# sweeneychris/TheiaSfM

Measured on AMD Instinct MI355X. Metric: ba_observations_per_sec, higher is better.
Workload: dtype f64

## Files before the change

### theiasfm_amd/csrc/device_view.h

```cpp
#pragma once
#include <cstdint>
#include <hip/hip_runtime.h>

namespace tmi {

constexpr int kSpmvTrips = 8;
constexpr unsigned kPinholeDefaultMask = 0x3Fu | (1u << 6) | (1u << 11) | (1u << 12);
constexpr int kWideK = 12;
constexpr int kWideKLarge = 20;
constexpr int kUltraK = 96;

struct DeviceView {
  int Nc, G, Np_pad, nslices, Nrb, D, DP;
  int n_ultra;
  int n_wide;
  int n_track_blocks;
  int Ncam_rb;
  int has_shared;
  int No_pad;
  int Nslots;
  int nub, nnzb;
  int n_order;
  long long npairs;

// ... 43 lines not shown
  const long long* pair_ptr;
  const int* pair_i;
  const int* pair_j;
  const int* ub_order;

  double* pm_r;
  double* pm_A;
  int drop_pos;
  double* pos_coef;
  double* xs;
  int compact;
  int sums_ready;
  double* cp_trk;
  double* xz;
  double* pm_Jp;
  double* pm_A1;
  int planes_fp32;
  double* cam_part;
  double* cm_Y;
  double* cm_A;
  double* cm_R;
  int direct_diag;
  double* trk_rec;
  double* scale_c;
  double* scale_cam;
  double* scale_p;
  double* prep;
  double* prep_c;
  double* Vinv;
  double* gp;
  double* Linv;
  double* Vraw;
  double* yp;
  double* red;
  double* Sdiag;
  double* tbuf;
  double* rbuf;
  double* Minv;
  double* rhs;
  double* yc;
  double* cg_r;
  double* cg_z;
  double* cg_p;
  double* cg_q;
  double* cg_t;
  double* partial;
  double* scal;
  int* flags;
  double* dotbuf;
  int* ticket;
  int* pcg_done;
};

struct HostMirror {
  double scal[32];
  double red[8];
  int flags[8];
  unsigned long long seq;
};

struct RedLayout {
  long long ub, diag, udiag, gt, gc, scalars, total;
};
inline RedLayout red_layout(long long nub, int Nrb, int D) {
  RedLayout L;
  L.ub = 0;
  L.diag = L.ub + nub * D * D;
  L.udiag = L.diag + (long long)Nrb * D * D;
  L.gt = L.udiag + (long long)Nrb * D;
  L.gc = L.gt + (long long)Nrb * D;
  L.scalars = L.gc + (long long)Nrb * D;
  L.total = L.scalars + 8;
  return L;
}

enum {
  SC_COST = 0,
  SC_SS = 1,
  SC_CAND_COST = 2,
  SC_CAND_SS = 3,
  SC_MCC = 4,
  SC_STEP_SQ = 5,
  SC_XNORM_SQ = 6,
  SC_GMAX = 7,
  SC_RHO = 8,
  SC_LAST_RHO = 9,
  SC_PQ = 10,
  SC_ALPHA = 11,
  SC_Q0 = 12,
  SC_Q1 = 13,
  SC_ZETA = 14,
  SC_BNORM = 15,
  SC_GMAX_P = 16,
  SC_RHO_BAD = 17,
  SC_II_DEXT = 18,
  SC_II_DINTR = 19,
  SC_II_XC = 22,
  SC_PCG_STOP = 24,
  SC_COUNT = 32
};
enum { FL_INVALID = 0, FL_SINGULAR_POINT = 1, FL_SINGULAR_BLOCK = 2, FL_PCG_FAIL = 3, FL_CHOL_ABORT = 4, FL_COUNT = 8 };

}
```

### theiasfm_amd/csrc/engine.hip

```cpp
#include <hip/hip_runtime.h>
#include <hip/hip_ext.h>
#include <dlfcn.h>

#include <algorithm>
#include <chrono>
#include <cmath>
#include <cstdio>
#include <cstring>
#include <functional>
#include <mutex>
#include <string>
#include <vector>

#include "../../include/theia_mi355_ba.h"
#include "dense_cholesky.h"
#include "dense_cholesky_df.h"
#include "cluster_chains.h"
#include "cluster_precond.h"
#include "kernels.h"
#include "mf_chunks.h"
#include "direct_diag.h"
#include "pcg_persist.h"
#include "track_kernels.h"
#include "relative_position_kernels.h"
// ... 388 lines not shown
  if (t < FL_COUNT) flags[t] = 0;
  if (t < 8) sc8[t] = 0.0;
}
__global__ void publish_kernel(const double* __restrict__ scal, const double* __restrict__ red8,
                               const int* __restrict__ flags, HostMirror* m, unsigned long long seq) {
  const int t = threadIdx.x;
  if (t < SC_COUNT) m->scal[t] = scal[t];
  if (t < 8) m->red[t] = red8[t];
  if (t < FL_COUNT) m->flags[t] = flags[t];
  __threadfence_system();
  __syncthreads();
  if (t == 0) __hip_atomic_store(&m->seq, seq, __ATOMIC_RELEASE, __HIP_MEMORY_SCOPE_SYSTEM);
}
__global__ void flag_to_scalar_kernel(const int* __restrict__ flag, double* __restrict__ dst) {
  if (threadIdx.x == 0) *dst = (*flag) ? 1.0 : 0.0;
}
}

struct tmi_ba_solver {
  Structure st;
  Launch launch;
  DeviceView v;
  RedLayout RL;
  int DP = 4;
  int device = 0;
  hipStream_t stream = nullptr;
  std::vector<void*> allocs;
  HostMirror* h_mirror = nullptr;
  HostMirror* d_mirror = nullptr;
  unsigned long long mirror_seq = 0;
  double* h_scal = nullptr;
  double* h_red = nullptr;
  int* h_flags = nullptr;
  std::vector<double> ext0, intr0, pts0;
  std::vector<int> grp_off_h;
  double *d_ext0 = nullptr, *d_intr0 = nullptr, *d_pts0 = nullptr;
  int n_intr = 0;
  double* d_pm_u = nullptr;
  double* d_cm_t = nullptr;
  bool need_slot_track = false;
  mfc::View mf = {};
  bool mf_ok = false;
  ddg::Plan dd = {};
  bool direct_ok = false;
  bool fuse_finish_ok = true;
  bool attach_events = true;
  bool pcg_speculate = true;
  bool fast_start_ok = true;
  bool compact_env = true;
  bool fuse_sums = true;
  bool compact_robust = true;
  bool cost_by_view = false;
  bool cost_warm = true;
  bool implicit = false;
  bool adaptive = false;
  bool implicit_now = false;
  bool y_records = false;
  int n_implicit_iterations = 0;
  int adaptive_break_even_override = -1;
  int adaptive_break_even = 4;
  double cur_inv_radius = 0.0;
  double time_vote = 0.0;
  const tmi_ba_options* cur_opts = nullptr;
  double* d_partial_max = nullptr;
  double* d_dense = nullptr;
  double* d_df_tiles = nullptr;
  double* d_df_linv = nullptr;
  int* d_df_flags = nullptr;
  int df_epoch = 0;
  int num_cus = 0;
  clp::Plan cl_plan;
  int shared_diag_chunks = 0;
  double* d_shared_diag_partial = nullptr;
  bool cluster_blocks = false;
  bool cl_built = false;
  int vis_type = 0;
  bool vis_clusters = false;
  std::vector<std::vector<int> > vis_members;
  std::vector<int> vis_cluster_of_rb;
  bool tri = false;
  chains::Segments tri_seg;
  bool cl_failed = false;
  bool cl_active = false;
  bool ppcg_ready = false, ppcg_off = false;
  int ppcg_grid = 0;
  double *d_ppcg_p = nullptr, *d_ppcg_x = nullptr, *d_ppcg_partial = nullptr;
  int* d_ppcg_bar = nullptr;
  long long* d_ppcg_prof = nullptr;
  bool cl_unavailable = false;
  bool cl_retired = false;
  clp::ClusterDesc* d_cl_desc = nullptr;
  clp::GatherEntry* d_cl_ge = nullptr;
  int* d_cl_idx = nullptr;
  double *d_cl_tiles = nullptr, *d_cl_linv = nullptr, *d_cl_vec = nullptr;
  int *d_cl_flags = nullptr, *d_cl_bad = nullptr;
  int cl_epoch = 0;
  int nblocks_slices = 0;
  int nblocks_tracks = 0;
  int nblocks_points = 0;
  tmi_ba_allreduce_fn allreduce = nullptr;
  void* allreduce_user = nullptr;
  void* nccl_comm = nullptr;
  unsigned prof_mask = 0;
  struct Ev { int cls; hipEvent_t a, b; };
  std::vector<Ev> events;
  size_t ev_used = 0;
// ... 50 lines not shown
  int4* d_view_cam = nullptr;
  bool view_index_ready = false;
  int n_order_dev = 0, n_spc_dev = 0;
};

namespace {


template <class T>
int dev_alloc(tmi_ba_solver* s, T** p, size_t n) {
  *p = nullptr;
  if (n == 0) n = 1;
  TMI_HIP(hipMalloc((void**)p, n * sizeof(T)));
  s->allocs.push_back((void*)*p);
  return TMI_BA_OK;
}
template <class T>
int dev_upload(tmi_ba_solver* s, T** p, const std::vector<T>& h) {
  int rc = dev_alloc(s, p, h.size());
  if (rc) return rc;
  if (!h.empty()) TMI_HIP(hipMemcpy(*p, h.data(), h.size() * sizeof(T), hipMemcpyHostToDevice));
  return TMI_BA_OK;
}

struct Timed {
  tmi_ba_solver* s;
  int cls;
  bool on;
  bool attached;
  tmi_ba_solver::Ev* ev = nullptr;
  Timed(tmi_ba_solver* s_, int cls_, bool attach = false) : s(s_), cls(cls_), attached(attach) {
    s->launches[cls]++;
    on = (s->prof_mask >> cls) & 1u;
    if (on) {
      if (s->ev_used == s->events.size()) {
        tmi_ba_solver::Ev e;
        e.cls = cls;
        hipEventCreate(&e.a);
        hipEventCreate(&e.b);
        s->events.push_back(e);
      }
      ev = &s->events[s->ev_used++];
      ev->cls = cls;
      if (!attached) hipEventRecord(ev->a, s->stream);
    }
  }
  hipEvent_t start() const { return on && attached ? ev->a : nullptr; }
  hipEvent_t stop() const { return on && attached ? ev->b : nullptr; }
  ~Timed() {
    if (on && !attached) hipEventRecord(ev->b, s->stream);
  }
};

void select_mirror(tmi_ba_solver* s, int slot) {
  s->h_scal = s->h_mirror[slot].scal;
  s->h_red = s->h_mirror[slot].red;
  s->h_flags = s->h_mirror[slot].flags;
}

int readback(tmi_ba_solver* s) {
  select_mirror(s, 0);
  const unsigned long long seq = ++s->mirror_seq;
  hipLaunchKernelGGL(publish_kernel, dim3(1), dim3(64), 0, s->stream, s->v.scal,
                     s->v.red + s->RL.scalars, s->v.flags, s->d_mirror, seq);
  volatile unsigned long long* p = &s->h_mirror->seq;
  for (unsigned spin = 1;; ++spin) {
    if (*p == seq) break;
    if ((spin & 0xfffu) == 0) {
      const hipError_t q = hipStreamQuery(s->stream);
      if (q == hipSuccess) break;
      if (q != hipErrorNotReady) {
        s->error = std::string("hipStreamQuery: ") + hipGetErrorString(q);
        return TMI_BA_ERR_DEVICE;
      }
    }
    __builtin_ia32_pause();
  }
  __atomic_thread_fence(__ATOMIC_ACQUIRE);
  const hipError_t le = hipGetLastError();
  if (le != hipSuccess) {
    s->error = std::string("kernel launch failed: ") + hipGetErrorString(le);
    return TMI_BA_ERR_DEVICE;
  }
  return TMI_BA_OK;
}

struct Rccl {
  struct Id { char b[128]; };
  int (*GetUniqueId)(void*) = nullptr;
  int (*CommInitRank)(void**, int, Id, int) = nullptr;
  int (*AllReduce)(const void*, void*, size_t, int, int, void*, hipStream_t) = nullptr;
  int (*CommDestroy)(void*) = nullptr;
  const char* (*GetErrorString)(int) = nullptr;
  bool ok = false;
  std::string error;
};
Rccl& rccl() {
  static Rccl r;
  static bool tried = false;
  if (tried) return r;
  tried = true;
  void* h = nullptr;
  const char* names[] = {"librccl.so", "librccl.so.1", "/opt/rocm/lib/librccl.so.1", "/opt/rocm/lib/librccl.so"};
  for (const char* n : names)
    if ((h = dlopen(n, RTLD_NOW | RTLD_NOLOAD))) break;
  if (!h)
// ... 1353 lines not shown
  TMI_HIP(hipMemsetAsync(v.pcg_done, 0, sizeof(int), s->stream));
  TMI_HIP(hipMemsetAsync(v.cg_q, 0, (size_t)(n_r + 8) * sizeof(double), s->stream));
  TMI_HIP(hipMemsetAsync(v.yc, 0, std::max(n_r, 1) * sizeof(double), s->stream));
  TMI_HIP(hipMemsetAsync(v.red, 0, s->RL.total * sizeof(double), s->stream));
  TMI_HIP(hipMemsetAsync(v.cm_Y, 0, (v.write_y ? (size_t)std::max<int64_t>(st.Nslots, 1) * YS : 1) * sizeof(double), s->stream));
  TMI_HIP(hipMemsetAsync(v.cm_A, 0, (size_t)std::max<int64_t>(st.Nslots, 1) * AS * sizeof(double), s->stream));
  {
    int* orb;
    if ((rc = dev_alloc(s, &orb, (size_t)std::max<int64_t>(st.No_pad, 1)))) return rc;
    if (st.No_pad > 0)
      hipLaunchKernelGGL(obs_rb_kernel, dim3((unsigned)((st.No_pad + 255) / 256)), dim3(256), 0, s->stream, v.obs_cam, v.cam_rb,
                         st.Nc, (long long)st.No_pad, orb);
    v.obs_rb = orb;
  }
  if (s->need_slot_track && !st.has_shared) {
    rc = build_mf_chunks(s);
    if (rc) return rc;
  }
  v.drop_pos = 0;
  const bool two_pass_possible = (s->implicit || s->adaptive) && !s->mf_ok;
  if (!light && !two_pass_possible && !st.has_shared && O->residual_precision != 32 && D >= 3 && s->DP >= 3) {
    const char* e = getenv("TMI_BA_DROP_POS");
    bool ok = !(e && atoi(e) == 0);
    for (int rb = 0; rb < st.Nrb && ok; ++rb) {
      const int c = st.rb_cam[rb];
      ok = c >= 0 && (st.cam_mask[c] & 7u) == 7u;
    }
    for (int lp = 0; lp < st.Np_pad && ok; ++lp) ok = st.pt_const[lp] == 0;
    if (ok) {
      if ((rc = dev_alloc(s, &v.pos_coef, (size_t)3 * std::max(st.Np_pad, 1)))) return rc;
      if ((rc = dev_alloc(s, &v.cp_trk, (size_t)7 * std::max(st.Np_pad, 1)))) return rc;
      if ((rc = dev_alloc(s, &v.xs, (size_t)std::max(st.Nrb, 1) * D + 8))) return rc;
      if ((rc = dev_alloc(s, &v.xz, (size_t)std::max(st.Nrb, 1) * D + 8))) return rc;
      v.drop_pos = 1;
    }
  }
  if (setup_timing) fprintf(stderr, "[tmi_ba setup] position columns of the A planes: %s\n", v.drop_pos ? "formed from Jp" : "stored");
  s->direct_ok = false;
  {
    const char* env = getenv("TMI_BA_FUSED_FINISH");
    s->fuse_finish_ok = !(env && env[0] == '0');
    env = getenv("TMI_BA_ATTACH_EVENTS");
    s->attach_events = !(env && env[0] == '0');
    env = getenv("TMI_BA_PCG_SPECULATE");
    s->pcg_speculate = !(env && env[0] == '0');
    env = getenv("TMI_BA_FAST_START");
    s->fast_start_ok = !(env && env[0] == '0');
    env = getenv("TMI_BA_COMPACT_PLANES");
    s->compact_env = !(env && env[0] == '0');
    env = getenv("TMI_BA_FUSE_TRACK_SUMS");
    s->fuse_sums = !(env && env[0] == '0');
    env = getenv("TMI_BA_COMPACT_ROBUST");
    s->compact_robust = !(env && env[0] == '0');
  }
  v.direct_diag = 0;
  {
    const char* e = getenv("TMI_BA_DIRECT_DIAG");
    if (s->mf_ok && !st.has_shared && O->residual_precision != 32 && !s->cluster_blocks && st.Nrb > 0 && st.Nslots > 0 && D <= ddg::kMaxD &&
        !(e && atoi(e) == 0)) {
      std::vector<int> cp((size_t)st.Nrb + 1);
      TMI_HIP(hipMemcpyAsync(cp.data(), v.cam_ptr, cp.size() * sizeof(int), hipMemcpyDeviceToHost, s->stream));
      TMI_HIP(hipStreamSynchronize(s->stream));
      std::vector<int> crb, cs0, cs1, rbc((size_t)st.Nrb + 1, 0);
      for (int rb = 0; rb < st.Nrb; ++rb) {
        rbc[rb] = (int)crb.size();
        const int n = cp[rb + 1] - cp[rb];
        if (n <= 0) continue;
        const int nch = (n + ddg::kChunkSlots - 1) / ddg::kChunkSlots;
        const int per = (((n + nch - 1) / nch) + 63) & ~63;
        for (int b = cp[rb]; b < cp[rb + 1]; b += per) {
          crb.push_back(rb);
          cs0.push_back(b);
          cs1.push_back(std::min(b + per, cp[rb + 1]));
        }
      }
      rbc[st.Nrb] = (int)crb.size();
      int *p0, *p1, *p2, *p3, *stt;
      double *xy, *part;
      if ((rc = dev_upload(s, &p0, crb))) return rc;
      if ((rc = dev_upload(s, &p1, cs0))) return rc;
      if ((rc = dev_upload(s, &p2, cs1))) return rc;
      if ((rc = dev_upload(s, &p3, rbc))) return rc;
      if ((rc = dev_alloc(s, &xy, (size_t)2 * st.Nslots))) return rc;
      if ((rc = dev_alloc(s, &part, std::max<size_t>(crb.size(), 1) * ddg::n_acc(D)))) return rc;
      if ((rc = dev_alloc(s, &v.trk_rec, (size_t)std::max(st.Np_pad, 1) * ddg::trk_stride(s->DP)))) return rc;
      if ((rc = dev_alloc(s, &stt, (size_t)st.Nslots))) return rc;
      hipLaunchKernelGGL(ddg::slot_gather_kernel, dim3(s->nblocks_tracks), dim3(256), 0, s->stream, v, stt, xy);
      v.slot_track = stt;
      s->dd.n_chunks = (int)crb.size();
      s->dd.chunk_rb = p0;
      s->dd.chunk_s0 = p1;
      s->dd.chunk_s1 = p2;
      s->dd.rb_chunk = p3;
      s->dd.cm_xy = xy;
      s->dd.part = part;
      s->direct_ok = true;
      const char* ec = getenv("TMI_BA_COST_BY_VIEW");
      if (const char* ew = getenv("TMI_BA_COST_WARM")) s->cost_warm = atoi(ew) != 0;
      s->cost_by_view = st.Nslots == st.No && ((int)crb.size() + 3) / 4 <= nbmax && !(ec && atoi(ec) == 0);
    }
  }
  if (s->adaptive) {
    const double form = (s->DP == 4 ? 79.0 : 61.0) * (double)st.npairs + (s->direct_ok ? 80.0 * (double)st.No : 0.0),
                 with_s = 195.0 * (double)st.nub,
                 free = (s->mf_ok ? (s->DP == 4 ? 57.0 : 52.0) : 85.0) * (double)st.No;
    if (const char* e = getenv("TMI_BA_BREAK_EVEN")) s->adaptive_break_even_override = atoi(e);
// ... 874 lines not shown
  hipStream_t stream = s->stream;
  s->prof_mask = (O->profile_kernels == 1) ? 0xffffffffu : (unsigned)O->profile_kernels;
  s->cl_retired = false;
  s->ev_used = 0;
  memset(s->launches, 0, sizeof(s->launches));
  sum->num_reduced_blocks = st.Nrb;
  sum->reduced_block_dim = D;
  sum->num_schur_blocks = st.nub + st.Nrb;
  sum->num_schur_pairs = st.npairs;
  sum->setup_time_in_seconds = s->setup_seconds;
  int rc;
#define CK(x) if ((rc = (x)) != TMI_BA_OK) return fail(rc)
#define CKH(call) do { hipError_t e_ = (call); if (e_ != hipSuccess) { s->error = std::string(#call) + ": " + hipGetErrorString(e_); return fail(TMI_BA_ERR_DEVICE); } } while (0)

  const int lt = O->loss_function_type;
  const double lw = O->robust_loss_width;
  const bool iterative = (O->linear_solver_type == TMI_BA_ITERATIVE_SCHUR || O->linear_solver_type == TMI_BA_CGNR);
  s->cur_opts = O;
  if (iterative && (s->st.has_shared || s->vis_clusters) &&
      ((s->tri && O->preconditioner_type == TMI_BA_PRECOND_CLUSTER_JACOBI) ||
       (!s->tri && O->preconditioner_type == TMI_BA_PRECOND_CLUSTER_TRIDIAGONAL && st.world == 1 && !s->implicit))) {
    s->error = "CLUSTER_JACOBI / CLUSTER_TRIDIAGONAL: the solver was created for the other one";
    return fail(TMI_BA_ERR_INVALID_ARGUMENT);
  }
  if (iterative && s->vis_clusters &&
      (O->preconditioner_type == TMI_BA_PRECOND_CLUSTER_JACOBI || O->preconditioner_type == TMI_BA_PRECOND_CLUSTER_TRIDIAGONAL) &&
      O->visibility_clustering_type != s->vis_type) {
    s->error = "visibility_clustering_type differs from the value the solver was created with";
    return fail(TMI_BA_ERR_INVALID_ARGUMENT);
  }
  if (s->implicit && !iterative) {
    s->error = "this solver was created for the implicit Schur operator (ITERATIVE_SCHUR); "
               "an exact linear solver type needs schur_mode = explicit at creation";
    return fail(TMI_BA_ERR_INVALID_ARGUMENT);
  }
  double* d_sc = v.red + RL.scalars;

  CKH(hipMemsetAsync(v.flags, 0, FL_COUNT * sizeof(int), stream));
  CKH(hipMemsetAsync(v.yc, 0, std::max(n_r, 1) * sizeof(double), stream));
  hipLaunchKernelGGL(fill_kernel, dim3((n_r + 255) / 256 + 1), dim3(256), 0, stream, v.scale_c, (long long)n_r, 1.0);
  s->launch.expand_scale(v, stream);
  prepare_cameras(s, v.ext, v.intr, v.prep);
  hipLaunchKernelGGL(fill_kernel, dim3((unsigned)(((long long)st.Np_pad * s->DP + 255) / 256 + 1)), dim3(256), 0, stream, v.scale_p, (long long)st.Np_pad * s->DP, 1.0);
  bool compact_possible = s->compact_env && v.drop_pos && v.uniform_pinhole_default && s->mf_ok && s->direct_ok && D == 9 &&
                          (lt == 0 || s->compact_robust) && iterative && !s->cluster_blocks && v.cp_trk != nullptr && !v.planes_fp32;
  if (compact_possible) {
    compact_possible = (int)s->grp_off_h.size() == st.G + 1;
    for (int g = 0; g < st.G && compact_possible; ++g) {
      const double* K = s->intr0.data() + s->grp_off_h[g];
      compact_possible = s->grp_off_h[g + 1] - s->grp_off_h[g] >= 7 && K[1] == 1.0 && K[2] == 0.0;
    }
  }
  int last_pcg_len = 0;
  auto linearize = [&](bool norms_only = false, bool full_planes = false) {
    if (!norms_only)
      v.compact = (!full_planes && compact_possible && (s->implicit || (s->adaptive && last_pcg_len <= s->adaptive_break_even)))
                      ? (lt == 0 ? 1 : 2)
                      : 0;
    if (!norms_only) v.sums_ready = (v.compact && s->fuse_sums) ? 1 : 0;
    Timed t(s, TMI_BA_K_LINEARIZE);
    s->launch.linearize(v, stream, v.prep, lt, lw, nbs, d_sc, norms_only ? 1 : 0);
  };
  v.direct_diag = (s->direct_ok && iterative) ? 1 : 0;
  const bool fast_start = O->jacobi_scaling && v.direct_diag && s->fast_start_ok;
  linearize(fast_start, O->jacobi_scaling != 0);
  hipLaunchKernelGGL(flag_to_scalar_kernel, dim3(1), dim3(64), 0, stream, v.flags + FL_INVALID, d_sc + 2);
  CK(do_allreduce(s, d_sc, 8));
  CK(readback(s));
  double hsc[8];
  memcpy(hsc, s->h_red, sizeof(hsc));
  const int64_t No_global_hint = st.No;
  (void)No_global_hint;
  if (hsc[2] > 0.0) {
    s->error = "residual evaluation failed at the start point (a track lies on a camera centre)";
    return fail(TMI_BA_ERR_EVALUATION_FAILED);
  }
  double cost = hsc[0];
  double n_obs_global = (double)st.No;
  if (st.world > 1) {
    double tmp[8] = {(double)st.No, 0, 0, 0, 0, 0, 0, 0};
    CKH(hipMemcpyAsync(d_sc, tmp, sizeof(tmp), hipMemcpyHostToDevice, stream));
    CK(do_allreduce(s, d_sc, 8));
    CKH(hipMemcpyAsync(tmp, d_sc, sizeof(tmp), hipMemcpyDeviceToHost, stream));
    CKH(hipStreamSynchronize(stream));
    n_obs_global = tmp[0];
  }
  sum->initial_cost = cost;
  sum->initial_rmse = n_obs_global > 0 ? std::sqrt(hsc[1] / n_obs_global) : 0.0;
  double final_ss = hsc[1];

  auto trial_cost = [&]() {
    if (s->cost_by_view) {
      const int nb = (s->dd.n_chunks + 3) / 4;
      hipLaunchKernelGGL(ddg::cost_view_kernel, dim3(nb), dim3(256), 0, stream, v, s->dd, v.prep_c, v.pts_c, lt, lw, FL_INVALID,
                         nb, v.partial, d_sc + 3, d_sc + 5, s->cost_warm ? 1 : 0);
    } else {
      s->launch.cost(v, stream, v.prep_c, v.pts_c, lt, lw, FL_INVALID, nbs, v.partial, d_sc + 3, d_sc + 5);
    }
  };
  auto build_camera_side = [&](double inv_radius, bool skip_direct_reduce = false) {
    {
      Timed t(s, TMI_BA_K_POINT_ELIMINATE);
      s->launch.point_eliminate(v, stream, inv_radius, O->min_lm_diagonal, O->max_lm_diagonal, nbs,
                                s->d_partial_max, d_sc + 6, O->gradient_tolerance, st.world > 1 ? d_sc + 0 : nullptr);
    }
    {
      Timed t(s, TMI_BA_K_CAMERA_DIAG);
      if (v.direct_diag) {
        s->launch.camera_diag_direct(v, stream, RL, s->dd, v.prep, lt, lw, skip_direct_reduce ? 1 : 0);
      } else {
        s->launch.camera_diag(v, stream, RL, s->shared_diag_chunks, s->d_shared_diag_partial);
        s->launch.shared_blocks(v, stream, RL);
      }
    }
  };
  if (O->jacobi_scaling) {
    if (fast_start) {
      Timed t(s, TMI_BA_K_CAMERA_DIAG);
      s->launch.track_records_points_only(v, stream, v.pts);
      s->launch.camera_diag_direct(v, stream, RL, s->dd, v.prep, lt, lw, 0);
    } else {
      {
        Timed t(s, TMI_BA_K_REDUCE);
        s->launch.point_scale(v, stream, nbs);
      }
      build_camera_side(1.0);
    }
    CK(do_allreduce(s, v.red + RL.udiag, n_r));
    {
      Timed t(s, TMI_BA_K_REDUCE);
      if (n_r) {
        CKH(hipMemcpyAsync(v.scale_c, v.red + RL.udiag, (size_t)n_r * sizeof(double), hipMemcpyDeviceToDevice, stream));
        hipLaunchKernelGGL(camera_scale_finish_kernel, dim3((n_r + 255) / 256), dim3(256), 0, stream, v.scale_c, n_r);
        s->launch.expand_scale(v, stream);
        prepare_cameras(s, v.ext, v.intr, v.prep);
      }
    }
    linearize();
  }
  double xnorm_cam_sq = 0.0, xnorm_pts_sq = 0.0;
  {
    Timed t(s, TMI_BA_K_UPDATE_COST);
    s->launch.update_cameras(v, stream, v.scal + SC_STEP_SQ, v.prep_c);
    hipLaunchKernelGGL(points_norm_kernel, dim3(nbp), dim3(256), 0, stream, v, v.pts, nbp, v.partial, d_sc);
  }
  CK(do_allreduce(s, d_sc, 8));
  CK(readback(s));
  memcpy(hsc, s->h_red, sizeof(hsc));
  xnorm_cam_sq = s->h_scal[SC_STEP_SQ + 1];
  xnorm_pts_sq = hsc[0];
  double x_norm = std::sqrt(xnorm_cam_sq + xnorm_pts_sq);

  const double t_loop = now_s();
  double radius = O->initial_trust_region_radius;
  double decrease_factor = 2.0;
  int invalid_run = 0;
  int iter = 0;
  int termination = 1;
  const char* why = "maximum number of iterations reached";
  int64_t pcg_iters = 0;
  s->n_implicit_iterations = 0;
  bool need_gradient_check = true;
  bool inner_enabled = O->use_inner_iterations != 0;
  bool time_up = false;

  for (;;) {
    if (iter >= O->max_num_iterations) break;
    if (st.world > 1 ? time_up : (now_s() - t_start >= O->max_solver_time_in_seconds)) {
      why = "maximum solver time reached";
      break;
    }
    ++iter;
    const double inv_radius = 1.0 / radius;
    const double radius_used = radius;
    const int64_t pcg_before = pcg_iters;
    auto trace = [&](double outcome, double cand, double mcc, double step) {
      if (!O->iteration_trace || iter > O->iteration_trace_capacity) return;
      double* row = O->iteration_trace + (size_t)(iter - 1) * TMI_BA_TRACE_STRIDE;
      row[0] = iter; row[1] = cost; row[2] = radius_used; row[3] = outcome; row[4] = cand; row[5] = mcc;
      row[6] = (double)(pcg_iters - pcg_before); row[7] = step;
    };
    hipLaunchKernelGGL(iteration_begin_kernel, dim3(1), dim3(64), 0, stream, v.flags, d_sc);
    s->cur_inv_radius = inv_radius;
    if (s->adaptive && iterative && !s->st.has_shared) {
      s->implicit_now = last_pcg_len <= s->adaptive_break_even;
      if (s->y_records) v.write_y = s->implicit_now ? 0 : 1;
      if (s->implicit_now) s->n_implicit_iterations++;
    } else if (s->implicit && iterative) {
      s->n_implicit_iterations++;
    }
    v.direct_diag = (s->direct_ok && iterative && s->implicit_now && !s->cluster_blocks) ? 1 : 0;
    if (v.compact && !v.direct_diag) {
      compact_possible = false;
      linearize();
      hipLaunchKernelGGL(iteration_begin_kernel, dim3(1), dim3(64), 0, stream, v.flags, d_sc);
    }
    const bool cluster_handle = s->st.has_shared || s->vis_clusters;
    const bool cluster_precond = O->preconditioner_type == TMI_BA_PRECOND_CLUSTER_JACOBI ||
                                 O->preconditioner_type == TMI_BA_PRECOND_CLUSTER_TRIDIAGONAL;
    const bool fuse_finish = s->fuse_finish_ok && iterative && n_r > 0 && !(cluster_handle && cluster_precond);
    const bool fuse_direct = fuse_finish && v.direct_diag && st.world == 1;
    build_camera_side(inv_radius, fuse_direct);
    if (!s->implicit_now || s->cluster_blocks) {
      Timed t(s, TMI_BA_K_SCHUR_OFFDIAG);
      s->launch.schur_offdiag(v, stream, RL);
      s->launch.cross_add(v, stream, RL);
    }
    CK(do_allreduce(s, v.red, RL.total));
    const int precond_mode = O->preconditioner_type == TMI_BA_PRECOND_IDENTITY ? 1
                             : O->preconditioner_type == TMI_BA_PRECOND_SCHUR_JACOBI_PARAMETER_BLOCKS ? 2 : 0;
    if (fuse_finish) {
      Timed t(s, TMI_BA_K_PRECONDITIONER);
      s->launch.camera_finish(v, stream, RL, s->dd, inv_radius, O->min_lm_diagonal, O->max_lm_diagonal,
                              need_gradient_check ? 1 : 0, precond_mode, fuse_direct ? 1 : 0);
      s->cl_active = false;
    } else {
      Timed t(s, TMI_BA_K_REDUCE);
// ... 14 lines not shown
            (void)hipGetLastError();
            s->error.clear();
            s->cl_unavailable = true;
            s->cl_active = false;
          } else if (rc != TMI_BA_OK) {
            return fail(rc);
          }
        }
      }
      const int64_t before = pcg_iters;
      if (s->cl_active && s->cl_failed) {
        usable = 0;
      } else {
        CK(solve_reduced_pcg(s, O, &usable, &pcg_iters, fuse_finish));
      }
      last_pcg_len = (int)(pcg_iters - before);
      sum->effective_preconditioner_type =
          s->cl_active ? (s->tri ? TMI_BA_PRECOND_CLUSTER_TRIDIAGONAL : TMI_BA_PRECOND_CLUSTER_JACOBI)
          : O->preconditioner_type == TMI_BA_PRECOND_IDENTITY ? TMI_BA_PRECOND_IDENTITY
          : O->preconditioner_type == TMI_BA_PRECOND_SCHUR_JACOBI_PARAMETER_BLOCKS ? TMI_BA_PRECOND_SCHUR_JACOBI_PARAMETER_BLOCKS
                                                                                    : TMI_BA_PRECOND_SCHUR_JACOBI;
    } else {
      CK(solve_reduced_dense(s, &usable));
    }
    if (!(iterative && n_r > 0)) {
      CK(readback(s));
      if (!iterative && s->h_flags[FL_CHOL_ABORT]) {
        TMI_HIP(hipMemsetAsync(v.flags + FL_CHOL_ABORT, 0, sizeof(int), stream));
        {
          Timed t(s, TMI_BA_K_CHOLESKY);
          CK(solve_reduced_dense_panels(s));
        }
        CK(readback(s));
      }
    }
    if (s->h_red[6] > 0.0 || s->h_flags[FL_SINGULAR_BLOCK]) usable = 0;
    if (need_gradient_check) {
      double vote = (s->h_scal[SC_GMAX] > O->gradient_tolerance) ? 1.0 : 0.0;
      if (st.world > 1)
        vote += s->h_red[0];
      else
        vote += (s->h_scal[SC_GMAX_P] > O->gradient_tolerance) ? 1.0 : 0.0;
      need_gradient_check = false;
      if (vote == 0.0) {
        termination = 0;
        why = "gradient tolerance reached";
        --iter;
        break;
      }
    }
    double model_cost_change = 0.0, step_sq = 0.0, cand_cost = 0.0, cand_ss = 0.0;
    double cand_xc_sq = 0.0, cand_xp_sq = 0.0;
    bool cand_invalid = false;
    if (usable) {
      {
        Timed t(s, TMI_BA_K_UPDATE_COST);
        s->launch.update_cameras(v, stream, v.scal + SC_STEP_SQ, v.prep_c);
      }
      {
        Timed t(s, TMI_BA_K_BACK_SUBSTITUTE);
        s->launch.back_substitute(v, stream, nbs, v.partial, d_sc + 0);
      }
      {
        Timed t(s, TMI_BA_K_UPDATE_COST);
        trial_cost();
      }
      if (st.world > 1 && now_s() - t_start >= O->max_solver_time_in_seconds) {
        s->time_vote = 1.0;
        CKH(hipMemcpyAsync(d_sc + 7, &s->time_vote, sizeof(double), hipMemcpyHostToDevice, stream));
      }
      CK(do_allreduce(s, d_sc, 8));
      CK(readback(s));
      memcpy(hsc, s->h_red, sizeof(hsc));
      time_up = st.world > 1 && hsc[7] > 0.0;
      model_cost_change = hsc[0];
      step_sq = hsc[1] + s->h_scal[SC_STEP_SQ];
      cand_xp_sq = hsc[2];
      cand_xc_sq = s->h_scal[SC_STEP_SQ + 1];
      cand_cost = hsc[3];
      cand_ss = hsc[4];
      cand_invalid = hsc[5] > 0.0;
      if (!(model_cost_change > 0.0)) usable = 0;
    }
    bool inner_useful = false;
    if (usable && inner_enabled && !cand_invalid) {
      CK(run_inner_sweep(s, O));
      {
        Timed t(s, TMI_BA_K_UPDATE_COST);
        CKH(hipMemsetAsync(v.flags + FL_INVALID, 0, sizeof(int), stream));
        prepare_cameras(s, v.ext_c, v.intr_c, v.prep_c);
        trial_cost();
        hipLaunchKernelGGL(diff_sq_kernel, dim3(1), dim3(1024), 0, stream, v.ext, v.ext_c, (long long)6 * st.Nc, v.scal + SC_II_DEXT);
        hipLaunchKernelGGL(diff_sq_kernel, dim3(1), dim3(1024), 0, stream, v.intr, v.intr_c, (long long)s->n_intr, v.scal + SC_II_DINTR);
        hipLaunchKernelGGL(points_diff_kernel, dim3(nbp), dim3(256), 0, stream, v, nbp, v.partial);
        hipLaunchKernelGGL(reduce_sum_kernel, dim3(2), dim3(256), 0, stream, v.partial, nbp, d_sc + 1);
        hipLaunchKernelGGL(cameras_norm_kernel, dim3(1), dim3(1024), 0, stream, v, v.scal + SC_II_XC);
      }
      CK(do_allreduce(s, d_sc, 8));
      CK(readback(s));
      const double inner_cost = s->h_red[3], inner_ss = s->h_red[4];
      if (s->h_red[5] > 0.0) {
        CKH(hipMemcpyAsync(v.ext_c, s->inner.bak_ext, (size_t)6 * st.Nc * sizeof(double), hipMemcpyDeviceToDevice, stream));
        if (s->n_intr) CKH(hipMemcpyAsync(v.intr_c, s->inner.bak_intr, (size_t)s->n_intr * sizeof(double), hipMemcpyDeviceToDevice, stream));
        CKH(hipMemcpyAsync(v.pts_c, s->inner.bak_pts, (size_t)4 * st.Np_pad * sizeof(double), hipMemcpyDeviceToDevice, stream));
        prepare_cameras(s, v.ext_c, v.intr_c, v.prep_c);
      } else {
        model_cost_change += cand_cost - inner_cost;
        inner_useful = inner_cost < cost;
        inner_enabled = (1.0 - inner_cost / cand_cost) > 1e-3;
        cand_cost = inner_cost;
        cand_ss = inner_ss;
        step_sq = s->h_scal[SC_II_DEXT] + s->h_scal[SC_II_DINTR] + s->h_red[1];
        cand_xc_sq = s->h_scal[SC_II_XC];
        cand_xp_sq = s->h_red[2];
        sum->num_inner_iteration_steps++;
      }
    }
    if (!usable) {
      trace(-1.0, std::nan(""), model_cost_change, 0.0);
      sum->num_unsuccessful_steps++;
      if (++invalid_run >= O->max_num_consecutive_invalid_steps) {
        termination = 2;
        why = "too many consecutive invalid steps";
        break;
      }
      radius /= decrease_factor;
      decrease_factor *= 2.0;
      if (radius < O->min_trust_region_radius) {
        termination = 0;
        why = "minimum trust region radius reached";
        break;
      }
      continue;
    }
    invalid_run = 0;
    if (cand_invalid) cand_cost = 1.7976931348623157e308;
    const double step_norm = std::sqrt(step_sq);
    if (step_norm <= O->parameter_tolerance * (x_norm + O->parameter_tolerance)) {
      trace(2.0, cand_cost, model_cost_change, step_norm);
      termination = 0;
      why = "parameter tolerance reached";
      break;
    }
    const double cost_change = cost - cand_cost;
    if (std::fabs(cost_change) <= O->function_tolerance * cost) {
      trace(3.0, cand_cost, model_cost_change, step_norm);
      termination = 0;
      why = "function tolerance reached";
      break;
    }
    const double relative_decrease = cost_change / model_cost_change;
    trace((inner_useful || relative_decrease > O->min_relative_decrease) ? 1.0 : 0.0, cand_cost, model_cost_change, step_norm);
    if (inner_useful || relative_decrease > O->min_relative_decrease) {
      std::swap(v.ext, v.ext_c);
      std::swap(v.intr, v.intr_c);
      std::swap(v.pts, v.pts_c);
      std::swap(v.prep, v.prep_c);
      cost = cand_cost;
      final_ss = cand_ss;
      x_norm = std::sqrt(cand_xc_sq + cand_xp_sq);
      sum->num_successful_steps++;
      radius = radius / std::fmax(1.0 / 3.0, 1.0 - std::pow(2.0 * relative_decrease - 1.0, 3));
      radius = std::fmin(O->max_trust_region_radius, radius);
      decrease_factor = 2.0;
      linearize();
      need_gradient_check = true;
    } else {
      sum->num_unsuccessful_steps++;
      radius /= decrease_factor;
      decrease_factor *= 2.0;
    }
    if (radius < O->min_trust_region_radius) {
      termination = 0;
      why = "minimum trust region radius reached";
      break;
    }
    if (O->verbose && st.rank == 0)
      fprintf(stderr, "[tmi_ba] it %3d cost %.10e radius %.3e pcg %lld\n", iter, cost, radius, (long long)pcg_iters);
  }
  CKH(hipStreamSynchronize(stream));
  const double t_end = now_s();
  (void)t_loop;

  sum->termination = termination;
  sum->num_iterations = iter;
  sum->num_linear_solver_iterations = pcg_iters;
  sum->num_matrix_free_iterations = s->n_implicit_iterations;
  sum->final_cost = cost;
  sum->final_rmse = n_obs_global > 0 ? std::sqrt(final_ss / n_obs_global) : 0.0;
  sum->success = (termination != 2);
  sum->status = (termination == 2) ? TMI_BA_ERR_LINEAR_SOLVER : TMI_BA_OK;
  sum->solve_time_in_seconds = t_end - t_start;
  set_message(sum, why);
  for (int c = 0; c < TMI_BA_NUM_KERNEL_CLASSES; ++c) sum->kernel_launches[c] = s->launches[c];
  for (size_t i = 0; i < s->ev_used; ++i) {
    float ms = 0.f;
    if (s->events[i].cls < 0) continue;
    if (hipEventElapsedTime(&ms, s->events[i].a, s->events[i].b) == hipSuccess)
      sum->kernel_seconds[s->events[i].cls] += 1e-3 * ms;
  }
  return sum->status;
#undef CK
#undef CKH
}

int32_t tmi_ba_solve(tmi_ba_problem* P, const tmi_ba_options* O, tmi_ba_summary* sum) {
  if (!P || !O || !sum) return TMI_BA_ERR_INVALID_ARGUMENT;
  tmi_ba_solver* s = nullptr;
  memset(sum, 0, sizeof(*sum));
  const int rc = tmi_ba_solver_create(P, O, 0, 1, &s);
  if (rc != TMI_BA_OK) {
    sum->status = rc;
    sum->termination = 2;
    set_message(sum, g_last_error.empty() ? tmi_ba_status_string(rc) : g_last_error.c_str());
    return rc;
  }
  const int rc2 = tmi_ba_solver_solve(s, O, sum);
  if (sum->success) tmi_ba_solver_download(s, P);
  tmi_ba_solver_destroy(s);
  return rc2;
// ... 1377 lines not shown
  int64_t psum = 0;
  for (int64_t k = 0; k < st.npairs; ++k)
    psum += (slot_obs[st.pair_i[k]] + 1) * 31 + (slot_obs[st.pair_j[k]] + 1) * 17;
  out[11] = psum;
  return TMI_BA_OK;
}

int32_t tmi_ba_solver_structure_checksums(tmi_ba_solver* s, uint64_t out[24]) {
  if (!s || !out) return TMI_BA_ERR_INVALID_ARGUMENT;
  TMI_HIP(hipSetDevice(s->device));
  TMI_HIP(hipStreamSynchronize(s->stream));
  const Structure& st = s->st;
  const DeviceView& v = s->v;
  auto sum = [&](const void* dev, size_t bytes, uint64_t* dst) -> int {
    std::vector<unsigned char> h(bytes);
    if (bytes) TMI_HIP(hipMemcpy(h.data(), dev, bytes, hipMemcpyDeviceToHost));
    uint64_t x = 1469598103934665603ULL;
    for (unsigned char c : h) x = (x ^ c) * 1099511628211ULL;
    *dst = x;
    return TMI_BA_OK;
  };
  int rc;
  memset(out, 0, 24 * sizeof(uint64_t));
  out[0] = s->device_structure ? 1 : 0;
  const size_t Npad = (size_t)st.Np_pad, Nop = (size_t)st.No_pad, Nrb = (size_t)st.Nrb, nub = (size_t)st.nub;
#define CS(i, ptr, n, T) if ((rc = sum(ptr, (size_t)(n) * sizeof(T), &out[i]))) return rc;
  CS(1, v.slice_ptr, st.nslices + 1, int) CS(2, v.pt_k, Npad, int) CS(3, v.pt_const, Npad, unsigned char)
  CS(4, v.obs_cam, Nop, int) CS(5, v.obs_xy, 2 * Nop, double) CS(6, v.obs_cpos, Nop, int)
  CS(7, v.cam_ptr, Nrb + 1, int) CS(20, s->d_pt_orig, Npad, int)
  if (!s->light && !s->implicit) {
    CS(8, v.ub_i, nub, int) CS(9, v.ub_j, nub, int) CS(10, v.urow_ptr, Nrb + 1, int) CS(11, v.ucol_ptr, Nrb + 1, int)
    CS(12, v.ucol_u, nub, int) CS(13, v.spc_row, v.n_spc, int) CS(14, v.spc_u0, v.n_spc, int)
    CS(15, v.spc_rptr, Nrb + 1, int) CS(16, v.pair_ptr, nub + 1, long long) CS(17, v.pair_i, st.npairs, int)
    CS(18, v.pair_j, st.npairs, int) CS(19, v.ub_order, (size_t)v.n_order * 4, int)
  }
#undef CS
  out[21] = (uint64_t)v.n_order;
  out[22] = (uint64_t)v.n_spc;
  out[23] = (uint64_t)st.Nslots;
  return TMI_BA_OK;
}

int32_t tmi_ba_solver_operator_info(tmi_ba_solver* s, int32_t out[8]) {
  if (!s || !out) return TMI_BA_ERR_INVALID_ARGUMENT;
  for (int i = 0; i < 8; ++i) out[i] = 0;
  out[0] = s->mf_ok ? 1 : 0;
  out[1] = s->v.drop_pos ? 1 : 0;
  out[2] = s->direct_ok ? 1 : 0;
  out[3] = s->adaptive ? 1 : 0;
  out[4] = s->implicit ? 1 : 0;
  out[5] = s->adaptive ? (int32_t)std::min(s->adaptive_break_even, 1 << 30) : 0;
  out[6] = ((s->st.has_shared || s->vis_clusters) && !s->cl_unavailable) ? 1 : 0;
  out[7] = s->v.compact ? 1 : 0;
  return TMI_BA_OK;
}

int32_t tmi_ba_solver_evaluate(tmi_ba_solver* s, double* residuals, double* jac_camera,
                               double* jac_shared, double* jac_point, uint8_t* valid,
                               int32_t* block_dim) {
  if (!s || s->light) return TMI_BA_ERR_INVALID_ARGUMENT;
  TMI_HIP(hipSetDevice(s->device));
  {
    const int rcm = materialize_host_layout(s);
    if (rcm) return rcm;
  }
  DeviceView& v = s->v;
  Structure& st = s->st;
  const int D = st.D, DP = s->DP;
  const int n_r = st.Nrb * D;
  hipStream_t stream = s->stream;
  if (block_dim) *block_dim = D;
  TMI_HIP(hipMemsetAsync(v.flags, 0, FL_COUNT * sizeof(int), stream));
  hipLaunchKernelGGL(fill_kernel, dim3((n_r + 255) / 256 + 1), dim3(256), 0, stream, v.scale_c, (long long)n_r, 1.0);
  s->launch.expand_scale(v, stream);
  prepare_cameras(s, v.ext, v.intr, v.prep);
  hipLaunchKernelGGL(fill_kernel, dim3((unsigned)(((long long)st.Np_pad * DP + 255) / 256 + 1)), dim3(256), 0, stream, v.scale_p, (long long)st.Np_pad * DP, 1.0);
  {
    DeviceView ve = v;
    ve.drop_pos = 0;
    ve.compact = 0;
    v.compact = 0;
    v.sums_ready = 0;
    s->launch.linearize(ve, stream, v.prep, 0, 1.0, s->nblocks_tracks, nullptr, 0);
  }
  const size_t N = (size_t)st.No_pad;
  std::vector<double> r(residuals ? 2 * N : 0), A(jac_camera ? (size_t)2 * D * N : 0),
      Jp(jac_point ? (size_t)2 * DP * N : 0);
  if (residuals) TMI_HIP(hipMemcpyAsync(r.data(), v.pm_r, r.size() * sizeof(double), hipMemcpyDeviceToHost, stream));
  if (jac_camera) TMI_HIP(hipMemcpyAsync(A.data(), v.pm_A, A.size() * sizeof(double), hipMemcpyDeviceToHost, stream));
  if (jac_point) TMI_HIP(hipMemcpyAsync(Jp.data(), v.pm_Jp, Jp.size() * sizeof(double), hipMemcpyDeviceToHost, stream));
  std::vector<double> A1((jac_shared && st.has_shared) ? (size_t)2 * D * N : 0);
  if (!A1.empty()) TMI_HIP(hipMemcpyAsync(A1.data(), v.pm_A1, A1.size() * sizeof(double), hipMemcpyDeviceToHost, stream));
  TMI_HIP(hipStreamSynchronize(stream));
  if (v.planes_fp32) {
    auto widen = [](std::vector<double>& buf) {
      std::vector<float> f(buf.size());
      if (!f.empty()) memcpy(f.data(), buf.data(), f.size() * sizeof(float));
      for (size_t k = 0; k < f.size(); ++k) buf[k] = (double)f[k];
    };
    widen(r); widen(A); widen(Jp); widen(A1);
  }
  for (size_t e = 0; e < N; ++e) {
    const int64_t i = st.obs_orig[e];
    if (i < 0) continue;
    auto at = [e](int npl, int plane) {
      return (e >> 6) * (size_t)(npl * 64) + (size_t)(plane >> 1) * 128 + ((e & 63) << 1) + (size_t)(plane & 1);
    };
    if (residuals) {
      residuals[2 * i] = r[at(2, 0)];
      residuals[2 * i + 1] = r[at(2, 1)];
    }
    if (jac_camera)
      for (int a = 0; a < D; ++a) {
        jac_camera[(size_t)2 * D * i + a] = A[at(2 * D, 2 * a)];
        jac_camera[(size_t)2 * D * i + D + a] = A[at(2 * D, 2 * a + 1)];
      }
    if (jac_shared)
      for (int a = 0; a < D; ++a) {
        jac_shared[(size_t)2 * D * i + a] = A1.empty() ? 0.0 : A1[at(2 * D, 2 * a)];
        jac_shared[(size_t)2 * D * i + D + a] = A1.empty() ? 0.0 : A1[at(2 * D, 2 * a + 1)];
      }
    if (jac_point)
      for (int a = 0; a < DP; ++a) {
        jac_point[(size_t)2 * DP * i + a] = Jp[at(2 * DP, 2 * a)];
        jac_point[(size_t)2 * DP * i + DP + a] = Jp[at(2 * DP, 2 * a + 1)];
      }
    if (valid) valid[i] = 1;
  }
  if (valid) {
// ... 24 lines not shown
```

### theiasfm_amd/lib.py

```python
from __future__ import annotations

import ctypes as C
import os

import numpy as np

from . import abi

_HERE = os.path.dirname(os.path.abspath(__file__))
LIB_PATH = os.path.join(_HERE, "lib", "libtheia_mi355_ba.so")
_lib = None

EXPORTS = (
    "tmi_ba_version", "tmi_ba_device_count", "tmi_ba_status_string", "tmi_ba_last_error",
    "tmi_ba_options_init",
    "tmi_ba_intrinsics_size", "tmi_ba_intrinsics_constant_mask", "tmi_ba_solve",
    "tmi_ba_solver_create", "tmi_ba_solver_set_allreduce", "tmi_ba_solver_solve",
    "tmi_ba_solver_reset", "tmi_ba_solver_set_parameters", "tmi_ba_solver_download", "tmi_ba_solver_stream",
    "tmi_ba_solver_destroy", "tmi_ba_solver_evaluate", "tmi_ba_structure_stats", "tmi_ba_structure_stats_for",
    "tmi_ba_rccl_unique_id", "tmi_ba_solver_init_rccl", "tmi_ba_solver_debug_allreduce",
    "tmi_ba_solver_filter_outlier_tracks", "tmi_ba_filter_outlier_tracks",
    "tmi_ba_solver_adjust_tracks", "tmi_ba_adjust_tracks",
    "tmi_ba_solver_adjust_views", "tmi_ba_adjust_views",
    "tmi_ba_track_estimator_options_init", "tmi_ba_solver_estimate_tracks", "tmi_ba_estimate_tracks",
# ... 425 lines not shown
            min_num_optimized_tracks_per_view, None if vm is None else vm.ctypes.data, sel.ctypes.data, ln.ctypes.data, err.ctypes.data,
            C.byref(ss))
        if st != 0:
            raise EngineError(st, "tmi_ba_solver_select_good_tracks")
        return sel, ln, err, ss

    def adjust_tracks(self, options: abi.COptions):
        n = self.problem.num_points
        term = np.full(n, -1, dtype=np.int8)
        iters = np.zeros(n, dtype=np.int32)
        c0 = np.zeros(n)
        c1 = np.zeros(n)
        ts = abi.CTrackBatchSummary()
        st = self._L.tmi_ba_solver_adjust_tracks(self._h, C.byref(options), term.ctypes.data,
                                                 iters.ctypes.data, c0.ctypes.data, c1.ctypes.data,
                                                 C.byref(ts))
        if st != 0:
            raise EngineError(st, "tmi_ba_solver_adjust_tracks")
        return term, iters, c0, c1, ts

    def adjust_views(self, options: abi.COptions, view_mask=None):
        vm, term, iters, c0, c1, vs = _view_outputs(self.problem.num_cameras, view_mask)
        st = self._L.tmi_ba_solver_adjust_views(self._h, C.byref(options), None if vm is None else vm.ctypes.data,
                                                term.ctypes.data, iters.ctypes.data, c0.ctypes.data, c1.ctypes.data,
                                                C.byref(vs))
        if st != 0:
            raise EngineError(st, "tmi_ba_solver_adjust_views")
        return term, iters, c0, c1, vs

    def estimate_tracks(self, estimator_options: abi.CTrackEstimatorOptions, ba_options: abi.COptions,
                        track_mask=None):
        tm, status, es = _track_mask(self.problem.num_points, track_mask)
        st = self._L.tmi_ba_solver_estimate_tracks(self._h, C.byref(estimator_options), C.byref(ba_options),
                                                   None if tm is None else tm.ctypes.data, status.ctypes.data,
                                                   C.byref(es))
        if st != 0:
            raise EngineError(st, "tmi_ba_solver_estimate_tracks")
        return status, es

    def structure_checksums(self):
        out = (C.c_uint64 * 24)()
        st = self._L.tmi_ba_solver_structure_checksums(self._h, out)
        if st != 0:
            raise EngineError(st, "tmi_ba_solver_structure_checksums")
        return list(out)

    def operator_info(self) -> dict:
        out = (C.c_int32 * 8)()
        st = self._L.tmi_ba_solver_operator_info(self._h, out)
        if st != 0:
            raise EngineError(st, "tmi_ba_solver_operator_info")
        return dict(one_sweep_product=bool(out[0]), position_columns_formed=bool(out[1]), direct_camera_side=bool(out[2]),
                    adaptive=bool(out[3]), implicit=bool(out[4]), break_even=int(out[5]), cluster_handle=bool(out[6]),
                    compact_planes=bool(out[7]))

    @property
    def stream(self) -> int:
        return int(self._L.tmi_ba_solver_stream(self._h) or 0)

    def evaluate(self, point_dof: int):
        n = self.problem.num_observations
        bd = C.c_int32(0)
        r = np.zeros((n, 2))
        A = np.zeros(n * 2 * 16)
        A1 = np.zeros(n * 2 * 16)
        Jp = np.zeros((n, 2, point_dof))
        valid = np.zeros(n, dtype=np.uint8)
        st = self._L.tmi_ba_solver_evaluate(self._h, r.ctypes.data, A.ctypes.data, A1.ctypes.data,
                                            Jp.ctypes.data, valid.ctypes.data, C.byref(bd))
        if st != 0:
            raise EngineError(st, "tmi_ba_solver_evaluate")
        D = bd.value
        return r, A[: n * 2 * D].reshape(n, 2, D), A1[: n * 2 * D].reshape(n, 2, D), Jp, valid, D

    def close(self):
        if self._h:
            self._L.tmi_ba_solver_destroy(self._h)
            self._h = C.c_void_p()

    def __del__(self):
        try:
            self.close()
        except Exception:
            pass
```

Before: 2.474 billion.

## Speculatively linearize at the candidate point into a second buffer set

When the step evaluation would use compact planes, the candidate cost is computed by a full linearization at the candidate parameters into a second set of residual/Jacobian/track buffers, instead of a separate trial-cost pass. If the step is accepted, the buffer sets are swapped, so the linearization after acceptance is not recomputed. The cost is extra device memory and wasted linearization work on rejected steps. It is gated on direct-diag mode, no inner iterations and the previous step having succeeded.

```diff
diff --git a/theiasfm_amd/csrc/device_view.h b/theiasfm_amd/csrc/device_view.h
--- a/theiasfm_amd/csrc/device_view.h
+++ b/theiasfm_amd/csrc/device_view.h
@@ -119,6 +119,24 @@
   int* pcg_done;
 };
 
+struct LinearisationSet {
+  double* pm_r;
+  double* pm_A;
+  double* pm_Jp;
+  double* cp_trk;
+  double* Vraw;
+  double* gp;
+};
+inline void swap_linearisation_set(DeviceView& v, LinearisationSet& o) {
+  double* t;
+  t = v.pm_r, v.pm_r = o.pm_r, o.pm_r = t;
+  t = v.pm_A, v.pm_A = o.pm_A, o.pm_A = t;
+  t = v.pm_Jp, v.pm_Jp = o.pm_Jp, o.pm_Jp = t;
+  t = v.cp_trk, v.cp_trk = o.cp_trk, o.cp_trk = t;
+  t = v.Vraw, v.Vraw = o.Vraw, o.Vraw = t;
+  t = v.gp, v.gp = o.gp, o.gp = t;
+}
+
 struct HostMirror {
   double scal[32];
   double red[8];
diff --git a/theiasfm_amd/csrc/engine.hip b/theiasfm_amd/csrc/engine.hip
--- a/theiasfm_amd/csrc/engine.hip
+++ b/theiasfm_amd/csrc/engine.hip
@@ -464,6 +464,10 @@
   bool compact_robust = true;
   bool cost_by_view = false;
   bool cost_warm = true;
+  bool spec_env = true;
+  bool spec_ready = false, spec_off = false;
+  bool spec_swapped = false;
+  LinearisationSet spec_set = {nullptr, nullptr, nullptr, nullptr, nullptr, nullptr};
   bool implicit = false;
   bool adaptive = false;
   bool implicit_now = false;
@@ -620,6 +624,32 @@
   }
 };
 
+void primary_linearisation_set(tmi_ba_solver* s) {
+  if (!s->spec_swapped) return;
+  swap_linearisation_set(s->v, s->spec_set);
+  s->spec_swapped = false;
+}
+bool ensure_speculative_set(tmi_ba_solver* s) {
+  if (s->spec_ready) return true;
+  if (s->spec_off) return false;
+  const size_t N = std::max<size_t>((size_t)s->st.No_pad, 1), NP = std::max<size_t>((size_t)s->st.Np_pad, 1);
+  const size_t DP = (size_t)s->DP, NS = (size_t)sym_size(s->DP);
+  const size_t n[6] = {2 * N, 4 * N, 2 * DP * N, 7 * NP, NS * NP, DP * NP};
+  double* p[6] = {nullptr, nullptr, nullptr, nullptr, nullptr, nullptr};
+  for (int i = 0; i < 6; ++i) {
+    if (hipMalloc((void**)&p[i], n[i] * sizeof(double)) != hipSuccess) {
+      (void)hipGetLastError();
+      for (int j = 0; j < i; ++j) (void)hipFree(p[j]);
+      s->spec_off = true;
+      return false;
+    }
+  }
+  for (int i = 0; i < 6; ++i) s->allocs.push_back((void*)p[i]);
+  s->spec_set = LinearisationSet{p[0], p[1], p[2], p[3], p[4], p[5]};
+  s->spec_ready = true;
+  return true;
+}
+
 void select_mirror(tmi_ba_solver* s, int slot) {
   s->h_scal = s->h_mirror[slot].scal;
   s->h_red = s->h_mirror[slot].red;
@@ -2079,6 +2109,8 @@
     s->fuse_sums = !(env && env[0] == '0');
     env = getenv("TMI_BA_COMPACT_ROBUST");
     s->compact_robust = !(env && env[0] == '0');
+    env = getenv("TMI_BA_SPECULATIVE_LINEARIZE");
+    s->spec_env = !(env && env[0] == '0');
   }
   v.direct_diag = 0;
   {
@@ -3059,11 +3091,17 @@
     }
   }
   int last_pcg_len = 0;
+  auto compact_now = [&](bool full_planes) {
+    return (!full_planes && compact_possible && (s->implicit || (s->adaptive && last_pcg_len <= s->adaptive_break_even)))
+               ? (lt == 0 ? 1 : 2)
+               : 0;
+  };
+  primary_linearisation_set(s);
   auto linearize = [&](bool norms_only = false, bool full_planes = false) {
-    if (!norms_only)
-      v.compact = (!full_planes && compact_possible && (s->implicit || (s->adaptive && last_pcg_len <= s->adaptive_break_even)))
-                      ? (lt == 0 ? 1 : 2)
-                      : 0;
+    if (!norms_only) {
+      v.compact = compact_now(full_planes);
+      if (!v.compact) primary_linearisation_set(s);
+    }
     if (!norms_only) v.sums_ready = (v.compact && s->fuse_sums) ? 1 : 0;
     Timed t(s, TMI_BA_K_LINEARIZE);
     s->launch.linearize(v, stream, v.prep, lt, lw, nbs, d_sc, norms_only ? 1 : 0);
@@ -3170,6 +3208,7 @@
   bool need_gradient_check = true;
   bool inner_enabled = O->use_inner_iterations != 0;
   bool time_up = false;
+  bool prev_step_ok = true;
 
   for (;;) {
     if (iter >= O->max_num_iterations) break;
@@ -3290,6 +3329,7 @@
     double model_cost_change = 0.0, step_sq = 0.0, cand_cost = 0.0, cand_ss = 0.0;
     double cand_xc_sq = 0.0, cand_xp_sq = 0.0;
     bool cand_invalid = false;
+    int spec_compact = 0;
     if (usable) {
       {
         Timed t(s, TMI_BA_K_UPDATE_COST);
@@ -3299,7 +3339,23 @@
         Timed t(s, TMI_BA_K_BACK_SUBSTITUTE);
         s->launch.back_substitute(v, stream, nbs, v.partial, d_sc + 0);
       }
-      {
+      spec_compact = 0;
+      if (s->spec_env && v.direct_diag && !O->use_inner_iterations && prev_step_ok) {
+        spec_compact = compact_now(false);
+        if (spec_compact && !ensure_speculative_set(s)) spec_compact = 0;
+      }
+      if (spec_compact) {
+        Timed t(s, TMI_BA_K_LINEARIZE);
+        DeviceView vs = v;
+        LinearisationSet other = s->spec_set;
+        swap_linearisation_set(vs, other);
+        vs.pts = v.pts_c;
+        vs.compact = spec_compact;
+        vs.sums_ready = s->fuse_sums ? 1 : 0;
+        CKH(hipMemsetAsync(v.flags + FL_INVALID, 0, sizeof(int), stream));
+        s->launch.linearize(vs, stream, v.prep_c, lt, lw, nbs, d_sc + 3, 0);
+        hipLaunchKernelGGL(flag_to_scalar_kernel, dim3(1), dim3(64), 0, stream, v.flags + FL_INVALID, d_sc + 5);
+      } else {
         Timed t(s, TMI_BA_K_UPDATE_COST);
         trial_cost();
       }
@@ -3357,6 +3413,7 @@
     if (!usable) {
       trace(-1.0, std::nan(""), model_cost_change, 0.0);
       sum->num_unsuccessful_steps++;
+      prev_step_ok = false;
       if (++invalid_run >= O->max_num_consecutive_invalid_steps) {
         termination = 2;
         why = "too many consecutive invalid steps";
@@ -3401,9 +3458,18 @@
       radius = radius / std::fmax(1.0 / 3.0, 1.0 - std::pow(2.0 * relative_decrease - 1.0, 3));
       radius = std::fmin(O->max_trust_region_radius, radius);
       decrease_factor = 2.0;
-      linearize();
+      if (spec_compact) {
+        swap_linearisation_set(v, s->spec_set);
+        s->spec_swapped = !s->spec_swapped;
+        v.compact = spec_compact;
+        v.sums_ready = s->fuse_sums ? 1 : 0;
+      } else {
+        linearize();
+      }
+      prev_step_ok = true;
       need_gradient_check = true;
     } else {
+      prev_step_ok = false;
       sum->num_unsuccessful_steps++;
       radius /= decrease_factor;
       decrease_factor *= 2.0;
@@ -4887,6 +4953,9 @@
   out[5] = s->adaptive ? (int32_t)std::min(s->adaptive_break_even, 1 << 30) : 0;
   out[6] = ((s->st.has_shared || s->vis_clusters) && !s->cl_unavailable) ? 1 : 0;
   out[7] = s->v.compact ? 1 : 0;
+  if (s->spec_env && !s->spec_off && s->compact_env && s->v.drop_pos && s->v.uniform_pinhole_default && s->mf_ok && s->direct_ok &&
+      s->st.D == 9 && s->v.cp_trk != nullptr && !s->v.planes_fp32 && !s->cluster_blocks)
+    out[7] |= 2;
   return TMI_BA_OK;
 }
 
@@ -4910,6 +4979,7 @@
   s->launch.expand_scale(v, stream);
   prepare_cameras(s, v.ext, v.intr, v.prep);
   hipLaunchKernelGGL(fill_kernel, dim3((unsigned)(((long long)st.Np_pad * DP + 255) / 256 + 1)), dim3(256), 0, stream, v.scale_p, (long long)st.Np_pad * DP, 1.0);
+  primary_linearisation_set(s);
   {
     DeviceView ve = v;
     ve.drop_pos = 0;
diff --git a/theiasfm_amd/lib.py b/theiasfm_amd/lib.py
--- a/theiasfm_amd/lib.py
+++ b/theiasfm_amd/lib.py
@@ -501,7 +501,7 @@
             raise EngineError(st, "tmi_ba_solver_operator_info")
         return dict(one_sweep_product=bool(out[0]), position_columns_formed=bool(out[1]), direct_camera_side=bool(out[2]),
                     adaptive=bool(out[3]), implicit=bool(out[4]), break_even=int(out[5]), cluster_handle=bool(out[6]),
-                    compact_planes=bool(out[7]))
+                    compact_planes=bool(out[7] & 1), speculative_linearize=bool(out[7] & 2))
 
     @property
     def stream(self) -> int:
```

Measured after the change: 2.526 billion (median of 6 runs). +2.1%, better.
